# hsp-iit/online-detection

Measured on AMD Instinct MI355X. Metric: FALKON fit+infer samples/sec (N=1e6 D=1024 M=1e4), higher is better.
Workload: dtype f32-accurate K_nM (X Z' as a two-term f16 split on the f16 MFMA, f32 accumulate) stored as 24-bit fixed point (step 2^-24) + f64 solver (preconditioner: K_MM, T and T^-1 in f64; the products of the A factor, which only preconditions, at f32 accuracy on the f16 MFMA)

## Files before the change

online-detection_amd/csrc/knm_pass_q.hip:

```cpp
#include <algorithm>
#include <stdlib.h>

#include "odx_internal.h"
#include "knm_q.h"

namespace odx {

template <int NT, int CH, int R, int NV, int FMT, int WPE>
__device__ __forceinline__ void knm_passq_body(const unsigned short* __restrict__ Khi, int64_t ldk,
                                               const unsigned char* __restrict__ Klo, int64_t ldlo, int64_t n,
                                               int64_t M, const double* __restrict__ v1, const double* __restrict__ v2,
                                               const double* __restrict__ w, double* __restrict__ slab, int64_t slab_ld,
                                               double* __restrict__ t_out, int wg, int nwg, int64_t Mv = 0,
                                               const int* __restrict__ cstart = nullptr, const int* __restrict__ cpos = nullptr) {
  constexpr int NW = NT / 64;
  constexpr int CW = QCW;
  extern __shared__ __attribute__((aligned(16))) double vsq[];
  __shared__ double red[2][NW][NV * R];
  const int tid = threadIdx.x, lane = tid & 63, wave = tid >> 6;
  const int nchunk = (int)((M + CW - 1) / CW);
  const int vcap = (nchunk + 1) * CW;
  const int64_t nblk = (n + R - 1) / R;
  const double vscale = FMT == QF_U24 ? 5.9604644775390625e-08 : 1.0;
  for (int i = tid; i < vcap; i += NT) {
    vsq[i] = (v1 != nullptr && i < M) ? q_v_entry(v1, i, Mv, cstart, cpos) * vscale : 0.0;
    if (NV == 2) vsq[vcap + i] = i < M ? q_v_entry(v2, i, Mv, cstart, cpos) * vscale : 0.0;
  }
  double acc[NV][CH][CW];
#pragma unroll
  for (int q = 0; q < NV; ++q)
#pragma unroll
    for (int c = 0; c < CH; ++c)
#pragma unroll
      for (int e = 0; e < CW; ++e) acc[q][c][e] = 0.0;

  QChunk<FMT, CW> kr[R][CH];
  const int rowb_hi = (int)ldk * 2, rowb_lo = (int)ldlo;
  const int voff_hi = tid * (2 * CW), voff_lo = tid * CW;
  __amdgpu_buffer_rsrc_t rs_hi, rs_lo;
  int rows_open = R;
  auto open_block = [&](int64_t blk) {
    const int64_t row0 = blk * R;
    rows_open = (int)(n - row0 < R ? n - row0 : R);
    rs_hi = __builtin_amdgcn_make_buffer_rsrc(const_cast<unsigned short*>(Khi + row0 * ldk), (short)0, rows_open * rowb_hi, 0x00020000);
    if (FMT == QF_U24)
      rs_lo = __builtin_amdgcn_make_buffer_rsrc(const_cast<unsigned char*>(Klo + row0 * ldlo), (short)0, rows_open * rowb_lo, 0x00020000);
  };
  auto load_block = [&](int c) {
#pragma unroll
    for (int r = 0; r < R; ++r) {
      const int rr = r < rows_open ? r : rows_open - 1;
      const u32x2q th = __builtin_amdgcn_raw_buffer_load_b64(rs_hi, voff_hi, rr * rowb_hi + c * (NT * 2 * CW), 0);
      kr[r][c].hi[0] = th[0], kr[r][c].hi[1] = th[1];
      if (FMT == QF_U24) kr[r][c].lo[0] = __builtin_amdgcn_raw_buffer_load_b32(rs_lo, voff_lo, rr * rowb_lo + c * (NT * CW), 0);
    }
  };

  int64_t blk = wg;
  if (blk < nblk) {
    open_block(blk);
#pragma unroll
    for (int c = 0; c < CH; ++c) load_block(c);
  }
  __syncthreads();
  int pp = 0;
  for (; blk < nblk; blk += nwg) {
    double t[NV][R];
#pragma unroll
    for (int q = 0; q < NV; ++q)
#pragma unroll
      for (int r = 0; r < R; ++r) t[q][r] = 0.0;
    if (v1 != nullptr) {
      int zofs;
      asm volatile("v_mov_b32 %0, 0" : "=v"(zofs));
#pragma unroll
      for (int c = 0; c < CH; ++c) {
#pragma unroll
        for (int q = 0; q < NV; ++q) {
          const int ch = tid + c * NT + zofs;
          const int vi = (ch < nchunk ? ch : nchunk) * CW;
          double vv[CW];
#pragma unroll
          for (int u = 0; u < CW / 2; ++u) {
            const f64x2q a = *reinterpret_cast<const f64x2q*>(&vsq[q * vcap + vi + 2 * u]);
            vv[2 * u] = a[0];
            vv[2 * u + 1] = a[1];
          }
#pragma unroll
          for (int r = 0; r < R; ++r)
#pragma unroll
            for (int e = 0; e < CW; ++e) t[q][r] = fma(q_entry<FMT, CW>(kr[r][c], e), vv[e], t[q][r]);
        }
        __builtin_amdgcn_sched_barrier(0);
      }
#pragma unroll
      for (int q = 0; q < NV; ++q)
#pragma unroll
        for (int r = 0; r < R; ++r) {
          double s = t[q][r];
#pragma unroll
          for (int off = 32; off > 0; off >>= 1) s += __shfl_xor(s, off);
          if (lane == 0) red[pp][wave][q * R + r] = s;
        }
      __syncthreads();
#pragma unroll
      for (int q = 0; q < NV; ++q)
#pragma unroll
        for (int r = 0; r < R; ++r) {
          double s = 0.0;
#pragma unroll
          for (int u = 0; u < NW; ++u) s += red[pp][u][q * R + r];
          t[q][r] = s;
        }
      pp ^= 1;
    }
    if (t_out != nullptr) {
      if (tid == 0) {
#pragma unroll
        for (int r = 0; r < R; ++r)
          if (blk * R + r < n) t_out[blk * R + r] = t[0][r];
      }
    }
#pragma unroll
    for (int r = 0; r < R; ++r) {
      const int64_t row = blk * R + r;
      if (row >= n) {
#pragma unroll
        for (int q = 0; q < NV; ++q) t[q][r] = 0.0;
      } else if (NV == 1 && w != nullptr) {
        t[0][r] += w[row];
      }
    }
#pragma unroll
    for (int c = 0; c < CH; ++c)
#pragma unroll
      for (int r = 0; r < R; ++r) {
#pragma unroll
        for (int u = 0; u < CW / 2; ++u) asm volatile("" : "+v"(kr[r][c].hi[u]));
        if (FMT == QF_U24) {
#pragma unroll
          for (int u = 0; u < CW / 4; ++u) asm volatile("" : "+v"(kr[r][c].lo[u]));
        }
      }
    const int64_t nxt = blk + nwg;
    if (nxt < nblk) open_block(nxt);
#pragma unroll
    for (int c = 0; c < CH; ++c) {
#pragma unroll
      for (int r = 0; r < R; ++r)
#pragma unroll
        for (int e = 0; e < CW; ++e) {
          const double kd = q_entry<FMT, CW>(kr[r][c], e);
#pragma unroll
          for (int q = 0; q < NV; ++q) acc[q][c][e] = fma(kd, t[q][r], acc[q][c][e]);
        }
      load_block(c);
      __builtin_amdgcn_sched_barrier(0);
    }
  }
  double* my = slab + (int64_t)wg * slab_ld * NV;
#pragma unroll
  for (int q = 0; q < NV; ++q)
#pragma unroll
    for (int c = 0; c < CH; ++c) {
      const int ch = tid + c * NT;
      if (ch < nchunk) {
#pragma unroll
        for (int e = 0; e < CW; ++e)
          if ((int64_t)ch * CW + e < slab_ld) my[q * slab_ld + (int64_t)ch * CW + e] = acc[q][c][e] * vscale;
      }
    }
}

template <int NT, int CH, int R, int NV, int FMT, int WPE>
__global__ __launch_bounds__(NT, WPE) void knm_passq_kernel(const unsigned short* __restrict__ Khi, int64_t ldk,
                                                       const unsigned char* __restrict__ Klo, int64_t ldlo, int64_t n,
                                                       int64_t M, const double* __restrict__ v1, const double* __restrict__ v2,
                                                       const double* __restrict__ w, double* __restrict__ slab, int64_t slab_ld,
                                                       double* __restrict__ t_out, int64_t Mv, const int* __restrict__ cstart,
                                                       const int* __restrict__ cpos) {
  knm_passq_body<NT, CH, R, NV, FMT, WPE>(Khi, ldk, Klo, ldlo, n, M, v1, v2, w, slab, slab_ld, t_out, (int)blockIdx.x, (int)gridDim.x, Mv,
                                          cstart, cpos);
}

struct PassBatchQ {
  const unsigned short* Khi[ODX_MAX_ZBATCH];
  const unsigned char* Klo[ODX_MAX_ZBATCH];
  int64_t ldk[ODX_MAX_ZBATCH];
  int64_t ldlo[ODX_MAX_ZBATCH];
  int64_t n[ODX_MAX_ZBATCH];
  int M[ODX_MAX_ZBATCH];
  int grid[ODX_MAX_ZBATCH];
};

template <int NT, int CH, int R, int FMT, int WPE = (NT >= 1024 ? 4 : 2)>
__global__ __launch_bounds__(NT, WPE) void knm_passq_batched_kernel(PassBatchQ pb, const double* __restrict__ v, int64_t vstride,
                                                                    double* __restrict__ slab, int64_t slab_ld, int64_t slab_stride) {
  const int b = blockIdx.y;
  if ((int)blockIdx.x >= pb.grid[b]) return;
  knm_passq_body<NT, CH, R, 1, FMT, WPE>(pb.Khi[b], pb.ldk[b], pb.Klo[b], pb.ldlo[b], pb.n[b], pb.M[b], v + (int64_t)b * vstride, nullptr,
                                         nullptr, slab + (int64_t)b * slab_stride, slab_ld, nullptr, (int)blockIdx.x, pb.grid[b]);
}

template <int CH, int R, int FMT>
__device__ __forceinline__ void knm_passq_stag_body(const unsigned short* __restrict__ Khi, int64_t ldk,
                                                    const unsigned char* __restrict__ Klo, int64_t ldlo, int64_t n,
                                                    int64_t M, const double* __restrict__ v1,
                                                    const double* __restrict__ w, double* __restrict__ slab,
                                                    int64_t slab_ld, double* __restrict__ t_out, int wg, int nwg,
                                                    int64_t Mv = 0, const int* __restrict__ cstart = nullptr,
                                                    const int* __restrict__ cpos = nullptr) {
  constexpr int NT = 256, CW = QCW;
  extern __shared__ __attribute__((aligned(16))) double vsq[];
  __shared__ double red[2][2][4][R];
  const int tid = threadIdx.x, lane = tid & 63;
  const int h = __builtin_amdgcn_readfirstlane(tid >> 8), hw = __builtin_amdgcn_readfirstlane((tid >> 6) & 3);
  const int ht = tid & 255;
  const int nchunk = (int)((M + CW - 1) / CW);
  constexpr int vcap = CH * NT * CW;
  const int64_t nblk = (n + R - 1) / R;
  const double vscale = FMT == QF_U24 ? 5.9604644775390625e-08 : 1.0;
  for (int i = tid; i < vcap; i += 512) vsq[i] = (v1 != nullptr && i < M) ? q_v_entry(v1, i, Mv, cstart, cpos) * vscale : 0.0;
  const int voff_hi = ht * (2 * CW), voff_lo = ht * CW;
  double acc[CH][CW];
#pragma unroll
  for (int c = 0; c < CH; ++c)
#pragma unroll
    for (int e = 0; e < CW; ++e) acc[c][e] = 0.0;
  QChunk<FMT, CW> kr[R][CH];
  const int rowb_hi = (int)ldk * 2, rowb_lo = (int)ldlo;
  __amdgpu_buffer_rsrc_t rs_hi, rs_lo;
  int rows_open = R;
  auto open_block = [&](int64_t blk) {
    const int64_t row0 = blk * R;
    rows_open = (int)(n - row0 < R ? n - row0 : R);
    rs_hi = __builtin_amdgcn_make_buffer_rsrc(const_cast<unsigned short*>(Khi + row0 * ldk), (short)0, rows_open * rowb_hi, 0x00020000);
    if (FMT == QF_U24)
      rs_lo = __builtin_amdgcn_make_buffer_rsrc(const_cast<unsigned char*>(Klo + row0 * ldlo), (short)0, rows_open * rowb_lo, 0x00020000);
  };
  auto load_block = [&](int c) {
#pragma unroll
    for (int r = 0; r < R; ++r) {
      const int rr = r < rows_open ? r : rows_open - 1;
      const u32x2q th = __builtin_amdgcn_raw_buffer_load_b64(rs_hi, voff_hi, rr * rowb_hi + c * (NT * 2 * CW), 0);
      kr[r][c].hi[0] = th[0], kr[r][c].hi[1] = th[1];
      if (FMT == QF_U24) kr[r][c].lo[0] = __builtin_amdgcn_raw_buffer_load_b32(rs_lo, voff_lo, rr * rowb_lo + c * (NT * CW), 0);
    }
  };
  __shared__ unsigned int arrived[2];
  if (tid < 2) arrived[tid] = 0u;
  const int64_t first = 2 * (int64_t)wg + h, step = 2 * (int64_t)nwg;
  const int64_t mine = first < nblk ? (nblk - first + step - 1) / step : 0;
  if (mine > 0) {
    open_block(first);
#pragma unroll
    for (int c = 0; c < CH; ++c) load_block(c);
  }
  __syncthreads();
  int pp = 0;
  for (int64_t k = 0; k < mine; ++k) {
    const int64_t blk = first + k * step;
    double t[R];
#pragma unroll
    for (int r = 0; r < R; ++r) t[r] = 0.0;
    if (v1 != nullptr) {
      int zofs;
      asm volatile("v_mov_b32 %0, 0" : "=v"(zofs));
#pragma unroll
      for (int c = 0; c < CH; ++c) {
        const int vi = (ht + c * NT + zofs) * CW;
        const f64x2q a = *reinterpret_cast<const f64x2q*>(&vsq[vi]);
        const f64x2q b = *reinterpret_cast<const f64x2q*>(&vsq[vi + 2]);
        const double v0 = a[0], v1_ = a[1], v2_ = b[0], v3 = b[1];
#pragma unroll
        for (int r = 0; r < R; ++r) {
          t[r] = fma(q_entry<FMT, CW>(kr[r][c], 0), v0, t[r]);
          t[r] = fma(q_entry<FMT, CW>(kr[r][c], 1), v1_, t[r]);
          t[r] = fma(q_entry<FMT, CW>(kr[r][c], 2), v2_, t[r]);
          t[r] = fma(q_entry<FMT, CW>(kr[r][c], 3), v3, t[r]);
        }
        __builtin_amdgcn_sched_barrier(0);
      }
#pragma unroll
      for (int r = 0; r < R; ++r) {
        double sum = t[r];
#pragma unroll
        for (int off = 32; off > 0; off >>= 1) sum += __shfl_xor(sum, off);
        if (lane == 0) red[h][pp][hw][r] = sum;
      }
      asm volatile("" ::: "memory");
      if (lane == 0) {
        __hip_atomic_fetch_add(&arrived[h], 1u, __ATOMIC_RELAXED, __HIP_MEMORY_SCOPE_WORKGROUP);
        const unsigned int want = 4u * (unsigned int)(k + 1);
        bool met = false;
        for (int spin = 0; spin < (1 << 26); ++spin) {
          if (__hip_atomic_load(&arrived[h], __ATOMIC_RELAXED, __HIP_MEMORY_SCOPE_WORKGROUP) >= want) { met = true; break; }
          __builtin_amdgcn_s_sleep(1);
        }
        if (!met) __builtin_trap();
      }
      __builtin_amdgcn_wave_barrier();
      asm volatile("" ::: "memory");
#pragma unroll
      for (int r = 0; r < R; ++r) t[r] = ((red[h][pp][0][r] + red[h][pp][1][r]) + red[h][pp][2][r]) + red[h][pp][3][r];
      pp ^= 1;
#pragma unroll
      for (int c = 0; c < CH; ++c)
#pragma unroll
        for (int r = 0; r < R; ++r) {
          asm volatile("" : "+v"(kr[r][c].hi[0]));
          asm volatile("" : "+v"(kr[r][c].hi[1]));
          if (FMT == QF_U24) asm volatile("" : "+v"(kr[r][c].lo[0]));
        }
    }
    if (t_out != nullptr && hw == 0) {
      if (lane == 0) {
#pragma unroll
        for (int r = 0; r < R; ++r)
          if (blk * R + r < n) t_out[blk * R + r] = t[r];
      }
    }
#pragma unroll
    for (int r = 0; r < R; ++r) {
      const int64_t row = blk * R + r;
      if (row >= n) t[r] = 0.0;
      else if (w != nullptr) t[r] += w[row];
    }
    const bool more = k + 1 < mine;
    if (more) open_block(blk + step);
#pragma unroll
    for (int c = 0; c < CH; ++c) {
#pragma unroll
      for (int r = 0; r < R; ++r)
#pragma unroll
        for (int e = 0; e < CW; ++e) acc[c][e] = fma(q_entry<FMT, CW>(kr[r][c], e), t[r], acc[c][e]);
      load_block(c);
      __builtin_amdgcn_sched_barrier(0);
    }
  }
  double* my = slab + (2 * (int64_t)wg + h) * slab_ld;
#pragma unroll
  for (int c = 0; c < CH; ++c) {
    const int ch = ht + c * NT;
    if (ch < nchunk) {
#pragma unroll
      for (int e = 0; e < CW; ++e)
        if ((int64_t)ch * CW + e < slab_ld) my[(int64_t)ch * CW + e] = acc[c][e] * vscale;
    }
  }
}

template <int CH, int R, int FMT>
__global__ __launch_bounds__(512, 2) void knm_passq_stag_kernel(const unsigned short* __restrict__ Khi, int64_t ldk,
                                                                const unsigned char* __restrict__ Klo, int64_t ldlo, int64_t n,
                                                                int64_t M, const double* __restrict__ v1,
                                                                const double* __restrict__ w, double* __restrict__ slab,
                                                                int64_t slab_ld, double* __restrict__ t_out, int64_t Mv,
                                                                const int* __restrict__ cstart, const int* __restrict__ cpos) {
  knm_passq_stag_body<CH, R, FMT>(Khi, ldk, Klo, ldlo, n, M, v1, w, slab, slab_ld, t_out, (int)blockIdx.x, (int)gridDim.x, Mv, cstart, cpos);
}

template <int CH, int R, int FMT>
__global__ __launch_bounds__(512, 2) void knm_passq_stag_batched_kernel(PassBatchQ pb, const double* __restrict__ v, int64_t vstride,
                                                                        double* __restrict__ slab, int64_t slab_ld,
                                                                        int64_t slab_stride) {
  const int b = blockIdx.y;
  if ((int)blockIdx.x >= pb.grid[b]) return;
  knm_passq_stag_body<CH, R, FMT>(pb.Khi[b], pb.ldk[b], pb.Klo[b], pb.ldlo[b], pb.n[b], pb.M[b], v + (int64_t)b * vstride, nullptr,
                                  slab + (int64_t)b * slab_stride, slab_ld, nullptr, (int)blockIdx.x, pb.grid[b]);
}

struct QCfg {
  int nt, ch, r, wg_per_cu;
};

static bool pick_qcfg(int64_t M, int nv, int fmt, QCfg* cfg) {
  const int64_t chunks = (M + 3) / 4;
  if (nv == 1) {
    if (chunks <= 256) { *cfg = {256, 1, 16, 2}; return true; }
    if (chunks <= 512) { *cfg = {0, 2, 8, 2}; return true; }
    if (chunks <= 1024) { *cfg = {0, 4, 4, 2}; return true; }
    if (chunks <= 2048) { *cfg = {256, 8, 3, 2}; return true; }
    if (chunks <= 2560) { *cfg = {0, 10, 2, 1}; return true; }
    if (chunks <= 3072) { *cfg = {512, 6, 4, 1}; return true; }
    if (chunks <= 5110) { *cfg = {1024, 5, 1, 1}; return true; }
    return false;
  }
  if (chunks <= 1024 || chunks > 2560) return false;
  if (chunks <= 2048) *cfg = {512, 4, 2, 1};
  else *cfg = {512, 5, 2, 1};
  const int64_t lds = 2 * (chunks + 1) * 4 * 8 + 2 * (cfg->nt / 64) * cfg->r * 2 * 8 + 64;
  return lds <= 163840;
}

static int g_pass_cus = 0;

int pass_cus() { return g_pass_cus > 0 ? g_pass_cus : workspace_cus(); }

static int qgrid_for(const QCfg& cfg, int64_t n) {
  const int cus = pass_cus();
  const int64_t nblk = cfg.nt == 0 ? ceil_div(ceil_div(n, cfg.r), 2) : ceil_div(n, cfg.r);
  int64_t g = (int64_t)cus * cfg.wg_per_cu;
  if (g > nblk) g = nblk;
  if (g < 1) g = 1;
  return (int)g;
}

template <int NV, int FMT>
static int dispatch_passq(const QCfg& cfg, const QBlock& b, int grid, size_t lds, hipStream_t s, const double* v, const double* v2,
                          const double* w, double* slab, int64_t slab_ld, double* t_out, const QCols& cm) {
#define ODX_Q(NT_, CH_, R_)                                                                                                      \
  return q_launch(knm_passq_kernel<NT_, CH_, R_, NV, FMT, (NT_ >= 1024 ? 4 : 2)>, dim3(grid), NT_, lds, s, b.hi, b.ldk, b.lo, b.ldlo, \
                  b.n, b.M, v, v2, w, slab, slab_ld, t_out, cm.Mv, cm.start, cm.pos)
#define ODX_QH(CH_, R_)                                                                                                          \
  return q_launch(knm_passq_stag_kernel<CH_, R_, FMT>, dim3(grid), 512, lds, s, b.hi, b.ldk, b.lo, b.ldlo, b.n, b.M, v, w, slab,  \
                  slab_ld, t_out, cm.Mv, cm.start, cm.pos)
  if constexpr (NV == 1) {
    if (cfg.nt == 0) {
      if (cfg.ch == 2) ODX_QH(2, 8);
      if (cfg.ch == 4) ODX_QH(4, 4);
      ODX_QH(10, 2);
    }
    if (cfg.nt == 256 && cfg.ch == 1) ODX_Q(256, 1, 16);
    if (cfg.nt == 256 && cfg.ch == 8) ODX_Q(256, 8, 3);
    if (cfg.nt == 512 && cfg.ch == 6) ODX_Q(512, 6, 4);
    ODX_Q(1024, 5, 1);
  } else {
    if (cfg.ch == 4) ODX_Q(512, 4, 2);
    ODX_Q(512, 5, 2);
  }
#undef ODX_Q
#undef ODX_QH
}

int check_q_block(const char* who, const void* K, int64_t ldk, const void* Klo, int64_t ldlo, int fmt, int64_t M) {
  ODX_REQUIRE(fmt == ODX_KNM_U24 || fmt == ODX_KNM_BF16, "%s: storage format must be ODX_KNM_U24 or ODX_KNM_BF16 (got %d)", who, fmt);
  ODX_REQUIRE(K && ldk % 8 == 0 && ldk >= round_up(M, 8) && (reinterpret_cast<uintptr_t>(K) & 7u) == 0,
              "%s: K must be 8-byte aligned with ldk %% 8 == 0, ldk >= roundup(M, 8)", who);
  if (fmt == ODX_KNM_U24)
    ODX_REQUIRE(Klo && ldlo % 8 == 0 && ldlo >= round_up(M, 8) && (reinterpret_cast<uintptr_t>(Klo) & 3u) == 0,
                "%s: the low-byte plane must be 4-byte aligned with ldlo %% 8 == 0, ldlo >= roundup(M, 8)", who);
  return ODX_OK;
}

static bool passq_batch_cfg(int B, const int64_t* M, int fmt, QCfg* out) {
  QCfg c0 = {0, 0, 0, 0};
  for (int b = 0; b < B; ++b) {
    QCfg c;
    if (M[b] <= 0 || !pick_qcfg(M[b], 1, fmt, &c)) return false;
    if (b == 0) c0 = c;
    else if (c.nt != c0.nt || c.ch != c0.ch || c.r != c0.r) return false;
  }
  const bool built = (c0.nt == 0 && (c0.ch == 2 || c0.ch == 4 || c0.ch == 10)) ||
                     (c0.nt == 256 && (c0.ch == 1 || c0.ch == 8)) || (c0.nt == 512 && c0.ch == 6);
  if (out) *out = c0;
  return B > 0 && built;
}

static void passq_batch_geometry(int B, const int64_t* n, const int64_t* M, const QCfg& cfg, int* gmax, int64_t* slab_ld) {
  int g = 1;
  int64_t mm = 1;
  for (int b = 0; b < B; ++b) {
    if (n[b] > 0) g = std::max(g, qgrid_for(cfg, n[b]));
    mm = std::max(mm, M[b]);
  }
  *gmax = g;
  *slab_ld = round_up(mm, 4);
}

int64_t knm_passq_batched_workspace_bytes(int B, const int64_t* n, const int64_t* M, int fmt) {
  QCfg cfg;
  if (!q_format(fmt) || !passq_batch_cfg(B, M, fmt, &cfg)) return ODX_ERR_UNSUPPORTED;
  int gmax;
  int64_t slab_ld;
  passq_batch_geometry(B, n, M, cfg, &gmax, &slab_ld);
  return (int64_t)B * (cfg.nt == 0 ? 2 : 1) * gmax * slab_ld * (int64_t)sizeof(double);
}

template <int FMT>
static int launch_passq_batched(const QCfg& cfg, const PassBatchQ& pb, int gmax, int B, size_t lds, hipStream_t s, const double* v,
                                int64_t vstride, double* slab, int64_t slab_ld, int64_t slab_stride) {
#define ODX_QB(NT_, CH_, R_) \
  return q_launch(knm_passq_batched_kernel<NT_, CH_, R_, FMT>, dim3(gmax, B), NT_, lds, s, pb, v, vstride, slab, slab_ld, slab_stride)
#define ODX_QBH(CH_, R_) \
  return q_launch(knm_passq_stag_batched_kernel<CH_, R_, FMT>, dim3(gmax, B), 512, lds, s, pb, v, vstride, slab, slab_ld, slab_stride)
  if (cfg.nt == 0 && cfg.ch == 2) ODX_QBH(2, 8);
  if (cfg.nt == 0 && cfg.ch == 4) ODX_QBH(4, 4);
  if (cfg.nt == 0 && cfg.ch == 10) ODX_QBH(10, 2);
  if (cfg.nt == 256 && cfg.ch == 1) ODX_QB(256, 1, 16);
  if (cfg.nt == 256 && cfg.ch == 8) ODX_QB(256, 8, 3);
  if (cfg.nt == 512 && cfg.ch == 6) ODX_QB(512, 6, 4);
#undef ODX_QB
#undef ODX_QBH
  set_error("knm_passq_batched: no class-batched kernel for this pass configuration");
  return ODX_ERR_UNSUPPORTED;
}

int knm_passq_batched(int B, const void* const* Khi, const int64_t* ldk, const void* const* Klo, const int64_t* ldlo, int fmt,
                      const int64_t* n, const int64_t* M, const double* v, int64_t vstride, double* out, int64_t ostride,
                      void* workspace, int64_t workspace_bytes, hipStream_t s) {
  ODX_REQUIRE(B >= 1 && B <= ODX_MAX_ZBATCH, "knm_passq_batched: 1..%d classes", ODX_MAX_ZBATCH);
  QCfg cfg;
  ODX_REQUIRE(q_format(fmt) && passq_batch_cfg(B, M, fmt, &cfg),
              "knm_passq_batched: the classes of a batch must share one pass configuration");
  int gmax;
  int64_t slab_ld;
  passq_batch_geometry(B, n, M, cfg, &gmax, &slab_ld);
  const int per = cfg.nt == 0 ? 2 : 1;
  const int64_t slab_stride = (int64_t)per * gmax * slab_ld;
  ODX_PROPAGATE(require_workspace("knm_passq_batched", workspace, workspace_bytes, (int64_t)B * slab_stride * (int64_t)sizeof(double)));
  PassBatchQ pb;
  int nslab[ODX_MAX_ZBATCH];
  for (int b = 0; b < ODX_MAX_ZBATCH; ++b) {
    const bool on = b < B;
    pb.Khi[b] = on ? static_cast<const unsigned short*>(Khi[b]) : nullptr;
    pb.Klo[b] = (on && fmt == ODX_KNM_U24) ? static_cast<const unsigned char*>(Klo[b]) : nullptr;
    pb.ldk[b] = on ? ldk[b] : 0;
    pb.ldlo[b] = (on && fmt == ODX_KNM_U24) ? ldlo[b] : 0;
    pb.n[b] = on ? n[b] : 0;
    pb.M[b] = on ? (int)M[b] : 0;
    pb.grid[b] = (on && n[b] > 0) ? qgrid_for(cfg, n[b]) : 0;
    nslab[b] = per * pb.grid[b];
    if (on && n[b] > 0) ODX_PROPAGATE(check_q_block("knm_passq_batched", Khi[b], ldk[b], Klo ? Klo[b] : nullptr, ldlo ? ldlo[b] : 0, fmt, M[b]));
  }
  double* slab = static_cast<double*>(workspace);
  const size_t lds = (cfg.nt == 0 ? (size_t)(cfg.ch * 256 * 4) : (size_t)(slab_ld + 4)) * sizeof(double);
  if (fmt == ODX_KNM_U24) ODX_PROPAGATE((launch_passq_batched<QF_U24>(cfg, pb, gmax, B, lds, s, v, vstride, slab, slab_ld, slab_stride)));
  else ODX_PROPAGATE((launch_passq_batched<QF_BF16>(cfg, pb, gmax, B, lds, s, v, vstride, slab, slab_ld, slab_stride)));
  ODX_CHECK_LAUNCH("knm_passq_batched");
  return slab_reduce_batched_f64(B, M, nslab, slab, slab_ld, slab_stride, out, ostride, s);
}

}

using namespace odx;

extern "C" const char* odx_knm_pass_kernel_name(int64_t M, int fmt, int nv) {
  static thread_local char name[96];
  name[0] = 0;
  if (fmt == 0) {
    snprintf(name, sizeof(name), nv == 2 ? "knm_pass2_kernel" : "knm_pass_kernel");
    return name;
  }
  QCfg cfg;
  if ((fmt != QF_U24 && fmt != QF_BF16) || (nv != 1 && nv != 2) || M <= 0 || !pick_qcfg(M, nv, fmt, &cfg)) return name;
  if (cfg.nt == 0) snprintf(name, sizeof(name), "knm_passq_stag_kernel<%d,%d,%d>", cfg.ch, cfg.r, fmt);
  else snprintf(name, sizeof(name), "knm_passq_kernel<%d,%d,%d,%d,%d,%d>", cfg.nt, cfg.ch, cfg.r, nv, fmt, cfg.nt >= 1024 ? 4 : 2);
  return name;
}

extern "C" int odx_set_pass_cus(int cus) {
  ODX_REQUIRE(cus >= 0 && cus <= 4096, "odx_set_pass_cus: 0 (the device's) .. 4096");
  g_pass_cus = cus;
  return ODX_OK;
}

extern "C" int64_t odx_knm_fwd_bwd_q_workspace_bytes(int64_t n, int64_t M, int fmt) {
  QCfg cfg;
  if (n <= 0 || M <= 0) return 0;
  if (!q_format(fmt) || !pick_qcfg(M, 1, fmt, &cfg)) return ODX_ERR_UNSUPPORTED;
  return (int64_t)workspace_cus() * (cfg.nt == 0 ? 2 * cfg.wg_per_cu : cfg.wg_per_cu) * round_up(M, 4) * (int64_t)sizeof(double);
}

static int check_q_cols(const char* who, const QCols& cm, int64_t M) {
  ODX_REQUIRE(cm.Mv >= M && cm.Mv <= INT32_MAX && cm.col_of && cm.start && cm.pos, "%s: needs Mv >= M and col_of, start, pos", who);
  return ODX_OK;
}

static int knm_fwd_bwd_q_impl(const void* K, int64_t ldk, const void* Klo, int64_t ldlo, int fmt, int64_t n, int64_t M,
                              const double* v, const double* w, double* out, double* t_out, void* workspace,
                              int64_t workspace_bytes, odx_stream_t stream, const QCols& cm = QCols()) {
  ODX_REQUIRE(M > 0 && out, "odx_knm_fwd_bwd_q: M <= 0 or null out");
  hipStream_t s = as_stream(stream);
  if (n <= 0) {
    ODX_CHECK_HIP(hipMemsetAsync(out, 0, (size_t)(cm.on() ? cm.Mv : M) * sizeof(double), s));
    return ODX_OK;
  }
  ODX_REQUIRE(v || w, "odx_knm_fwd_bwd_q: both v and w null");
  ODX_PROPAGATE(check_q_block("odx_knm_fwd_bwd_q", K, ldk, Klo, ldlo, fmt, M));
  QCfg cfg;
  if (!pick_qcfg(M, 1, fmt, &cfg)) {
    set_error("odx_knm_fwd_bwd_q: M = %lld exceeds the %lld columns the compact-format pass kernels are built for", (long long)M,
              (long long)Q_MAX_M);
    return ODX_ERR_UNSUPPORTED;
  }
  const int grid = qgrid_for(cfg, n);
  const int64_t slab_ld = round_up(M, 4);
  const int nslab = cfg.nt == 0 ? 2 * grid : grid;
  ODX_PROPAGATE(require_workspace("odx_knm_fwd_bwd_q", workspace, workspace_bytes, (int64_t)nslab * slab_ld * (int64_t)sizeof(double)));
  double* slab = static_cast<double*>(workspace);
  const size_t lds = (cfg.nt == 0 ? (size_t)(cfg.ch * 256 * 4) : (size_t)(slab_ld + 4)) * sizeof(double);
  ODX_PROPAGATE(q_dispatch(q_block(K, ldk, Klo, ldlo, fmt, n, M), [&](auto f, const QBlock& b) {
    return dispatch_passq<1, decltype(f)::value>(cfg, b, grid, lds, s, v, nullptr, w, slab, slab_ld, t_out, cm);
  }));
  ODX_CHECK_LAUNCH("odx_knm_fwd_bwd_q");
  if (cm.on()) return slab_reduce_cols_f64(slab, slab_ld, nslab, 1, M, cm.Mv, cm.col_of, out, nullptr, s);
  return slab_reduce_f64(slab, slab_ld, nslab, M, out, s);
}

extern "C" int odx_knm_fwd_bwd_q(const void* K, int64_t ldk, const void* Klo, int64_t ldlo, int fmt, int64_t n, int64_t M,
                                 const double* v, const double* w, double* out, void* workspace, int64_t workspace_bytes,
                                 odx_stream_t stream) {
  return knm_fwd_bwd_q_impl(K, ldk, Klo, ldlo, fmt, n, M, v, w, out, nullptr, workspace, workspace_bytes, stream);
}

extern "C" int odx_knm_fwd_bwd_q_t(const void* K, int64_t ldk, const void* Klo, int64_t ldlo, int fmt, int64_t n, int64_t M,
                                   const double* v, const double* w, double* out, double* t_out, void* workspace,
                                   int64_t workspace_bytes, odx_stream_t stream) {
  ODX_REQUIRE(t_out == nullptr || v != nullptr, "odx_knm_fwd_bwd_q_t: t_out needs v");
  return knm_fwd_bwd_q_impl(K, ldk, Klo, ldlo, fmt, n, M, v, w, out, t_out, workspace, workspace_bytes, stream);
}

extern "C" int64_t odx_knm_fwd_bwd2_q_workspace_bytes(int64_t n, int64_t M, int fmt) {
  QCfg cfg;
  if (n <= 0 || M <= 0) return 0;
  if (!q_format(fmt) || !pick_qcfg(M, 2, fmt, &cfg)) return ODX_ERR_UNSUPPORTED;
  return 2 * (int64_t)workspace_cus() * cfg.wg_per_cu * round_up(M, 4) * (int64_t)sizeof(double);
}

static int knm_fwd_bwd2_q_impl(const void* K, int64_t ldk, const void* Klo, int64_t ldlo, int fmt, int64_t n, int64_t M,
                               const double* v, const double* v2, double* out, double* out2, double* t_out, void* workspace,
                               int64_t workspace_bytes, odx_stream_t stream, const QCols& cm = QCols()) {
  ODX_REQUIRE(M > 0 && out && out2, "odx_knm_fwd_bwd2_q: M <= 0 or null out");
  hipStream_t s = as_stream(stream);
  if (n <= 0) {
    ODX_CHECK_HIP(hipMemsetAsync(out, 0, (size_t)(cm.on() ? cm.Mv : M) * sizeof(double), s));
    ODX_CHECK_HIP(hipMemsetAsync(out2, 0, (size_t)(cm.on() ? cm.Mv : M) * sizeof(double), s));
    return ODX_OK;
  }
  ODX_REQUIRE(v && v2, "odx_knm_fwd_bwd2_q: null v or v2");
  ODX_PROPAGATE(check_q_block("odx_knm_fwd_bwd2_q", K, ldk, Klo, ldlo, fmt, M));
  QCfg cfg;
  if (!pick_qcfg(M, 2, fmt, &cfg)) {
    set_error("odx_knm_fwd_bwd2_q: M = %lld is outside the two-vector configurations (use two single passes)", (long long)M);
    return ODX_ERR_UNSUPPORTED;
  }
  const int grid = qgrid_for(cfg, n);
  const int64_t slab_ld = round_up(M, 4);
  ODX_PROPAGATE(require_workspace("odx_knm_fwd_bwd2_q", workspace, workspace_bytes, 2 * (int64_t)grid * slab_ld * (int64_t)sizeof(double)));
  double* slab = static_cast<double*>(workspace);
  const size_t lds = (size_t)(2 * (slab_ld + 4) * sizeof(double));
  ODX_PROPAGATE(q_dispatch(q_block(K, ldk, Klo, ldlo, fmt, n, M), [&](auto f, const QBlock& b) {
    return dispatch_passq<2, decltype(f)::value>(cfg, b, grid, lds, s, v, v2, nullptr, slab, slab_ld, t_out, cm);
  }));
  ODX_CHECK_LAUNCH("odx_knm_fwd_bwd2_q");
  if (cm.on()) return slab_reduce_cols_f64(slab, slab_ld, grid, 2, M, cm.Mv, cm.col_of, out, out2, s);
  return slab_reduce2_f64(slab, slab_ld, grid, M, out, out2, s);
}

extern "C" int odx_knm_fwd_bwd2_q(const void* K, int64_t ldk, const void* Klo, int64_t ldlo, int fmt, int64_t n, int64_t M,
                                  const double* v, const double* v2, double* out, double* out2, void* workspace,
                                  int64_t workspace_bytes, odx_stream_t stream) {
  return knm_fwd_bwd2_q_impl(K, ldk, Klo, ldlo, fmt, n, M, v, v2, out, out2, nullptr, workspace, workspace_bytes, stream);
}

extern "C" int odx_knm_fwd_bwd2_q_t(const void* K, int64_t ldk, const void* Klo, int64_t ldlo, int fmt, int64_t n, int64_t M,
                                    const double* v, const double* v2, double* out, double* out2, double* t_out, void* workspace,
                                    int64_t workspace_bytes, odx_stream_t stream) {
  return knm_fwd_bwd2_q_impl(K, ldk, Klo, ldlo, fmt, n, M, v, v2, out, out2, t_out, workspace, workspace_bytes, stream);
}

extern "C" int odx_knm_fwd_bwd_q_cols_t(const void* K, int64_t ldk, const void* Klo, int64_t ldlo, int fmt, int64_t n, int64_t M,
                                        const double* v, const double* w, double* out, double* t_out, void* workspace,
                                        int64_t workspace_bytes, int64_t Mv, const int32_t* col_of, const int32_t* start,
                                        const int32_t* pos, odx_stream_t stream) {
  ODX_REQUIRE(t_out == nullptr || v != nullptr, "odx_knm_fwd_bwd_q_cols_t: t_out needs v");
  const QCols cm = {Mv, col_of, start, pos};
  ODX_PROPAGATE(check_q_cols("odx_knm_fwd_bwd_q_cols_t", cm, M));
  return knm_fwd_bwd_q_impl(K, ldk, Klo, ldlo, fmt, n, M, v, w, out, t_out, workspace, workspace_bytes, stream, cm);
}

extern "C" int odx_knm_fwd_bwd2_q_cols_t(const void* K, int64_t ldk, const void* Klo, int64_t ldlo, int fmt, int64_t n, int64_t M,
                                         const double* v, const double* v2, double* out, double* out2, double* t_out,
                                         void* workspace, int64_t workspace_bytes, int64_t Mv, const int32_t* col_of,
                                         const int32_t* start, const int32_t* pos, odx_stream_t stream) {
  const QCols cm = {Mv, col_of, start, pos};
  ODX_PROPAGATE(check_q_cols("odx_knm_fwd_bwd2_q_cols_t", cm, M));
  return knm_fwd_bwd2_q_impl(K, ldk, Klo, ldlo, fmt, n, M, v, v2, out, out2, t_out, workspace, workspace_bytes, stream, cm);
}
```

online-detection_amd/csrc/knm_q.h:

```cpp
#pragma once
#include <type_traits>

#include "odx_internal.h"

namespace odx {

typedef unsigned int u32x4q __attribute__((ext_vector_type(4)));
typedef unsigned int u32x2q __attribute__((ext_vector_type(2)));
typedef double f64x2q __attribute__((ext_vector_type(2)));

enum { QF_U24 = 1, QF_BF16 = 2 };

constexpr int QCW = 4;
template <int FMT, int CW>
struct QChunk {
  unsigned hi[CW / 2];
  unsigned lo[CW / 4];
};

template <int FMT, int CW>
__device__ __forceinline__ double q_entry(const QChunk<FMT, CW>& k, int e) {
  const unsigned h = k.hi[e >> 1];
  if (FMT == QF_U24) {
    const unsigned sel = ((e & 1) ? 0x0c070600u : 0x0c050400u) | (unsigned)(e & 3);
    return (double)__builtin_amdgcn_perm(h, k.lo[e >> 2], sel);
  }
  return (double)__uint_as_float((e & 1) ? (h & 0xffff0000u) : (h << 16));
}

struct QCols {
  int64_t Mv = 0;
  const int* col_of = nullptr;
  const int* start = nullptr;
  const int* pos = nullptr;
  bool on() const { return start != nullptr; }
};

__device__ __forceinline__ double cols_fold_entry(const double* __restrict__ v, int64_t d, int64_t Mv, const int* __restrict__ start,
                                                  const int* __restrict__ pos) {
  const int last = (int)Mv - 1;
  int k = start[d], e = start[d + 1];
  k = k < 0 ? 0 : k;
  e = e > (int)Mv ? (int)Mv : e;
  double s = 0.0;
  for (; k < e; ++k) {
    int j = pos[k];
    j = j < 0 ? 0 : (j > last ? last : j);
    s += v[j];
  }
  return s;
}

__device__ __forceinline__ double q_v_entry(const double* __restrict__ v, int64_t i, int64_t Mv, const int* __restrict__ start,
                                            const int* __restrict__ pos) {
  return start == nullptr ? v[i] : cols_fold_entry(v, i, Mv, start, pos);
}

struct QBlock {
  const unsigned short* hi;
  int64_t ldk;
  const unsigned char* lo;
  int64_t ldlo;
  int fmt;
  int64_t n, M;
};

inline QBlock q_block(const void* K, int64_t ldk, const void* Klo, int64_t ldlo, int fmt, int64_t n, int64_t M) {
  return {static_cast<const unsigned short*>(K), ldk, static_cast<const unsigned char*>(Klo), ldlo, fmt, n, M};
}

inline bool q_format(int fmt) { return fmt == ODX_KNM_U24 || fmt == ODX_KNM_BF16; }

template <typename F>
int q_dispatch(QBlock b, F&& f) {
  if (b.fmt == ODX_KNM_U24) return f(std::integral_constant<int, QF_U24>(), b);
  b.lo = nullptr, b.ldlo = 0;
  return f(std::integral_constant<int, QF_BF16>(), b);
}

template <typename... P, typename... A>
int q_launch(void (*kernel)(P...), dim3 grid, int threads, size_t lds, hipStream_t s, A... args) {
  if (lds > 0)
    ODX_CHECK_HIP(hipFuncSetAttribute(reinterpret_cast<const void*>(kernel), hipFuncAttributeMaxDynamicSharedMemorySize, (int)lds));
  hipLaunchKernelGGL(kernel, grid, dim3(threads), lds, s, args...);
  return ODX_OK;
}

constexpr int64_t Q_MAX_M = 20440;
inline int q_nvt(int nv) { return nv <= 2 ? 2 : nv <= 4 ? 4 : 8; }
inline bool q_nv_supported(int64_t M, int fmt, int nv) { return q_format(fmt) && M > 0 && M <= Q_MAX_M && nv >= 1 && nv <= 8; }
#define ODX_REQUIRE_Q_NV(who, M, fmt, nv)                                                                                          \
  do {                                                                                                                             \
    if (!q_nv_supported(M, fmt, nv)) {                                                                                             \
      set_error("%s: needs ODX_KNM_U24 or ODX_KNM_BF16, 1 <= M <= %lld and 1 <= nv <= 8 (got fmt %d, M %lld, nv %d)", who,         \
                (long long)Q_MAX_M, fmt, (long long)(M), nv);                                                                      \
      return ODX_ERR_UNSUPPORTED;                                                                                                  \
    }                                                                                                                              \
  } while (0)

inline int workspace_cus() {
  const int cus = odx_device_cus();
  return cus > 0 ? cus : 256;
}

inline int require_workspace(const char* who, const void* workspace, int64_t workspace_bytes, int64_t need) {
  if (workspace != nullptr && workspace_bytes >= need) return ODX_OK;
  set_error("%s: workspace too small", who);
  return ODX_ERR_WORKSPACE;
}

inline int reduce_nv(int nv, int64_t M, int nslab, const double* slab, int64_t slab_ld, double* out, int64_t ldo, hipStream_t s) {
  int64_t Ms[8];
  int ns[8];
  for (int q = 0; q < nv; ++q) Ms[q] = M, ns[q] = nslab;
  return slab_reduce_batched_f64(nv, Ms, ns, slab, slab_ld, (int64_t)nslab * slab_ld, out, ldo, s);
}

}
```

Measured before the change: 193,600.

## Route two-vector K_nM pass with large M through staggered two-half kernel

For the NV=2, CH=5 configuration (M between 8192 and ~10240 columns), the pass kernel now dispatches to the staggered body, generalized to two vectors. The workgroup splits into two 256-thread halves that walk interleaved runs of 8 rows. Each half covers the full M range with 10 chunks per thread and skips chunks past the end. The two halves' accumulators are merged through LDS before the slab write, and t_out rows are batched per 8-row run. This aims to raise per-row parallelism and latency hiding in the dominant K_nM pass, at the cost of extra LDS, a final cross-half reduction, and more register pressure.

After: 193,900, median of 6. Within noise of the previous version (+0.1%).

```diff
diff --git a/online-detection_amd/csrc/knm_pass_q.hip b/online-detection_amd/csrc/knm_pass_q.hip
--- a/online-detection_amd/csrc/knm_pass_q.hip
+++ b/online-detection_amd/csrc/knm_pass_q.hip
@@ -172,17 +172,6 @@
     }
 }
 
-template <int NT, int CH, int R, int NV, int FMT, int WPE>
-__global__ __launch_bounds__(NT, WPE) void knm_passq_kernel(const unsigned short* __restrict__ Khi, int64_t ldk,
-                                                       const unsigned char* __restrict__ Klo, int64_t ldlo, int64_t n,
-                                                       int64_t M, const double* __restrict__ v1, const double* __restrict__ v2,
-                                                       const double* __restrict__ w, double* __restrict__ slab, int64_t slab_ld,
-                                                       double* __restrict__ t_out, int64_t Mv, const int* __restrict__ cstart,
-                                                       const int* __restrict__ cpos) {
-  knm_passq_body<NT, CH, R, NV, FMT, WPE>(Khi, ldk, Klo, ldlo, n, M, v1, v2, w, slab, slab_ld, t_out, (int)blockIdx.x, (int)gridDim.x, Mv,
-                                          cstart, cpos);
-}
-
 struct PassBatchQ {
   const unsigned short* Khi[ODX_MAX_ZBATCH];
   const unsigned char* Klo[ODX_MAX_ZBATCH];
@@ -202,31 +191,41 @@
                                          nullptr, slab + (int64_t)b * slab_stride, slab_ld, nullptr, (int)blockIdx.x, pb.grid[b]);
 }
 
-template <int CH, int R, int FMT>
+template <int CH, int R, int FMT, int NV = 1, int LOCH = 0>
 __device__ __forceinline__ void knm_passq_stag_body(const unsigned short* __restrict__ Khi, int64_t ldk,
                                                     const unsigned char* __restrict__ Klo, int64_t ldlo, int64_t n,
-                                                    int64_t M, const double* __restrict__ v1,
+                                                    int64_t M, const double* __restrict__ v1, const double* __restrict__ v2,
                                                     const double* __restrict__ w, double* __restrict__ slab,
                                                     int64_t slab_ld, double* __restrict__ t_out, int wg, int nwg,
                                                     int64_t Mv = 0, const int* __restrict__ cstart = nullptr,
                                                     const int* __restrict__ cpos = nullptr) {
   constexpr int NT = 256, CW = QCW;
+  constexpr int G = NV == 1 ? 1 : QRUN / R;
+  static_assert(NV == 1 || (G * R == QRUN && (G & (G - 1)) == 0), "a run is 8 rows: R must be 1, 2, 4 or 8");
+  constexpr int SURE = NV == 1 ? CH : LOCH / NT;
   extern __shared__ __attribute__((aligned(16))) double vsq[];
-  __shared__ double red[2][2][4][R];
+  __shared__ double red[2][2][4][NV * R];
+  __shared__ double trow[2][QRUN];
   const int tid = threadIdx.x, lane = tid & 63;
   const int h = __builtin_amdgcn_readfirstlane(tid >> 8), hw = __builtin_amdgcn_readfirstlane((tid >> 6) & 3);
   const int ht = tid & 255;
   const int nchunk = (int)((M + CW - 1) / CW);
-  constexpr int vcap = CH * NT * CW;
+  const int vcap = NV == 1 ? CH * NT * CW : (nchunk + 1) * CW;
   const int64_t nblk = (n + R - 1) / R;
   const double vscale = FMT == QF_U24 ? 5.9604644775390625e-08 : 1.0;
-  for (int i = tid; i < vcap; i += 512) vsq[i] = (v1 != nullptr && i < M) ? q_v_entry(v1, i, Mv, cstart, cpos) * vscale : 0.0;
+  for (int i = tid; i < vcap; i += 512) {
+    vsq[i] = (v1 != nullptr && i < M) ? q_v_entry(v1, i, Mv, cstart, cpos) * vscale : 0.0;
+    if (NV == 2) vsq[vcap + i] = i < M ? q_v_entry(v2, i, Mv, cstart, cpos) * vscale : 0.0;
+  }
   const int voff_hi = ht * (2 * CW), voff_lo = ht * CW;
-  double acc[CH][CW];
-#pragma unroll
-  for (int c = 0; c < CH; ++c)
-#pragma unroll
-    for (int e = 0; e < CW; ++e) acc[c][e] = 0.0;
+  double acc[NV][CH][CW];
+#pragma unroll
+  for (int q = 0; q < NV; ++q)
+#pragma unroll
+    for (int c = 0; c < CH; ++c)
+#pragma unroll
+      for (int e = 0; e < CW; ++e) acc[q][c][e] = 0.0;
+  auto walks = [&](int c) { return c < SURE || hw * 64 + c * NT < nchunk; };
   QChunk<FMT, CW> kr[R][CH];
   const int rowb_hi = (int)ldk * 2, rowb_lo = (int)ldlo;
   __amdgpu_buffer_rsrc_t rs_hi, rs_lo;
@@ -249,45 +248,74 @@
   };
   __shared__ unsigned int arrived[2];
   if (tid < 2) arrived[tid] = 0u;
+  const int64_t nrun = (nblk + G - 1) / G;
   const int64_t first = 2 * (int64_t)wg + h, step = 2 * (int64_t)nwg;
-  const int64_t mine = first < nblk ? (nblk - first + step - 1) / step : 0;
+  const int64_t runs = first < nrun ? (nrun - first + step - 1) / step : 0;
+  const int64_t mine = runs * G - ((runs > 0 && first + (runs - 1) * step == nrun - 1) ? nrun * G - nblk : 0);
+  auto block_of = [&](int64_t k) { return (first + (k / G) * step) * G + (k & (G - 1)); };
   if (mine > 0) {
-    open_block(first);
+    open_block(block_of(0));
 #pragma unroll
     for (int c = 0; c < CH; ++c) load_block(c);
   }
   __syncthreads();
   int pp = 0;
   for (int64_t k = 0; k < mine; ++k) {
-    const int64_t blk = first + k * step;
-    double t[R];
-#pragma unroll
-    for (int r = 0; r < R; ++r) t[r] = 0.0;
+    const int64_t blk = block_of(k);
+    double t[NV][R];
+#pragma unroll
+    for (int q = 0; q < NV; ++q)
+#pragma unroll
+      for (int r = 0; r < R; ++r) t[q][r] = 0.0;
     if (v1 != nullptr) {
       int zofs;
       asm volatile("v_mov_b32 %0, 0" : "=v"(zofs));
 #pragma unroll
       for (int c = 0; c < CH; ++c) {
-        const int vi = (ht + c * NT + zofs) * CW;
-        const f64x2q a = *reinterpret_cast<const f64x2q*>(&vsq[vi]);
-        const f64x2q b = *reinterpret_cast<const f64x2q*>(&vsq[vi + 2]);
-        const double v0 = a[0], v1_ = a[1], v2_ = b[0], v3 = b[1];
+        if constexpr (NV == 1) {
+          const int vi = (ht + c * NT + zofs) * CW;
+          const f64x2q a = *reinterpret_cast<const f64x2q*>(&vsq[vi]);
+          const f64x2q b = *reinterpret_cast<const f64x2q*>(&vsq[vi + 2]);
+          const double v0 = a[0], v1_ = a[1], v2_ = b[0], v3 = b[1];
+#pragma unroll
+          for (int r = 0; r < R; ++r) {
+            t[0][r] = fma(q_entry<FMT, CW>(kr[r][c], 0), v0, t[0][r]);
+            t[0][r] = fma(q_entry<FMT, CW>(kr[r][c], 1), v1_, t[0][r]);
+            t[0][r] = fma(q_entry<FMT, CW>(kr[r][c], 2), v2_, t[0][r]);
+            t[0][r] = fma(q_entry<FMT, CW>(kr[r][c], 3), v3, t[0][r]);
+          }
+        } else if (walks(c)) {
+          const int ch = ht + c * NT + zofs;
+          const int vi = (ch < nchunk ? ch : nchunk) * CW;
+          double vv[NV][CW];
+#pragma unroll
+          for (int q = 0; q < NV; ++q)
+#pragma unroll
+            for (int u = 0; u < CW / 2; ++u) {
+              const f64x2q a = *reinterpret_cast<const f64x2q*>(&vsq[q * vcap + vi + 2 * u]);
+              vv[q][2 * u] = a[0];
+              vv[q][2 * u + 1] = a[1];
+            }
+#pragma unroll
+          for (int r = 0; r < R; ++r)
+#pragma unroll
+            for (int e = 0; e < CW; ++e) {
+              const double kd = q_entry<FMT, CW>(kr[r][c], e);
+#pragma unroll
+              for (int q = 0; q < NV; ++q) t[q][r] = fma(kd, vv[q][e], t[q][r]);
+            }
+        }
+        __builtin_amdgcn_sched_barrier(0);
+      }
+#pragma unroll
+      for (int q = 0; q < NV; ++q)
 #pragma unroll
         for (int r = 0; r < R; ++r) {
-          t[r] = fma(q_entry<FMT, CW>(kr[r][c], 0), v0, t[r]);
-          t[r] = fma(q_entry<FMT, CW>(kr[r][c], 1), v1_, t[r]);
-          t[r] = fma(q_entry<FMT, CW>(kr[r][c], 2), v2_, t[r]);
-          t[r] = fma(q_entry<FMT, CW>(kr[r][c], 3), v3, t[r]);
-        }
-        __builtin_amdgcn_sched_barrier(0);
-      }
-#pragma unroll
-      for (int r = 0; r < R; ++r) {
-        double sum = t[r];
-#pragma unroll
-        for (int off = 32; off > 0; off >>= 1) sum += __shfl_xor(sum, off);
-        if (lane == 0) red[h][pp][hw][r] = sum;
-      }
+          double sum = t[q][r];
+#pragma unroll
+          for (int off = 32; off > 0; off >>= 1) sum += __shfl_xor(sum, off);
+          if (lane == 0) red[h][pp][hw][q * R + r] = sum;
+        }
       asm volatile("" ::: "memory");
       if (lane == 0) {
         __hip_atomic_fetch_add(&arrived[h], 1u, __ATOMIC_RELAXED, __HIP_MEMORY_SCOPE_WORKGROUP);
@@ -302,7 +330,12 @@
       __builtin_amdgcn_wave_barrier();
       asm volatile("" ::: "memory");
 #pragma unroll
-      for (int r = 0; r < R; ++r) t[r] = ((red[h][pp][0][r] + red[h][pp][1][r]) + red[h][pp][2][r]) + red[h][pp][3][r];
+      for (int q = 0; q < NV; ++q)
+#pragma unroll
+        for (int r = 0; r < R; ++r) {
+          const int i = q * R + r;
+          t[q][r] = ((red[h][pp][0][i] + red[h][pp][1][i]) + red[h][pp][2][i]) + red[h][pp][3][i];
+        }
       pp ^= 1;
 #pragma unroll
       for (int c = 0; c < CH; ++c)
@@ -313,40 +346,111 @@
           if (FMT == QF_U24) asm volatile("" : "+v"(kr[r][c].lo[0]));
         }
     }
-    if (t_out != nullptr && hw == 0) {
+    if constexpr (G == 1) {
+      if (t_out != nullptr && hw == 0) {
+        if (lane == 0) {
+#pragma unroll
+          for (int r = 0; r < R; ++r)
+            if (blk * R + r < n) t_out[blk * R + r] = t[0][r];
+        }
+      }
+    } else if (t_out != nullptr && hw == 0) {
+      const int g = (int)(k & (G - 1));
       if (lane == 0) {
 #pragma unroll
-        for (int r = 0; r < R; ++r)
-          if (blk * R + r < n) t_out[blk * R + r] = t[r];
+        for (int r = 0; r < R; ++r) trow[h][g * R + r] = t[0][r];
+      }
+      if (g == G - 1 || k + 1 == mine) {
+        asm volatile("" ::: "memory");
+        const int64_t row = (blk - g) * R + lane;
+        if (lane < QRUN && row < n) t_out[row] = trow[h][lane];
       }
     }
 #pragma unroll
     for (int r = 0; r < R; ++r) {
       const int64_t row = blk * R + r;
-      if (row >= n) t[r] = 0.0;
-      else if (w != nullptr) t[r] += w[row];
+      if (row >= n) {
+#pragma unroll
+        for (int q = 0; q < NV; ++q) t[q][r] = 0.0;
+      } else if (NV == 1 && w != nullptr) {
+        t[0][r] += w[row];
+      }
     }
     const bool more = k + 1 < mine;
-    if (more) open_block(blk + step);
+    if (more) open_block(block_of(k + 1));
 #pragma unroll
     for (int c = 0; c < CH; ++c) {
-#pragma unroll
-      for (int r = 0; r < R; ++r)
-#pragma unroll
-        for (int e = 0; e < CW; ++e) acc[c][e] = fma(q_entry<FMT, CW>(kr[r][c], e), t[r], acc[c][e]);
+      if (walks(c)) {
+#pragma unroll
+        for (int r = 0; r < R; ++r)
+#pragma unroll
+          for (int e = 0; e < CW; ++e) {
+            const double kd = q_entry<FMT, CW>(kr[r][c], e);
+#pragma unroll
+            for (int q = 0; q < NV; ++q) acc[q][c][e] = fma(kd, t[q][r], acc[q][c][e]);
+          }
+      }
       load_block(c);
       __builtin_amdgcn_sched_barrier(0);
     }
   }
-  double* my = slab + (2 * (int64_t)wg + h) * slab_ld;
-#pragma unroll
-  for (int c = 0; c < CH; ++c) {
-    const int ch = ht + c * NT;
-    if (ch < nchunk) {
-#pragma unroll
-      for (int e = 0; e < CW; ++e)
-        if ((int64_t)ch * CW + e < slab_ld) my[(int64_t)ch * CW + e] = acc[c][e] * vscale;
-    }
+  if constexpr (NV == 1) {
+    double* my = slab + (2 * (int64_t)wg + h) * slab_ld;
+#pragma unroll
+    for (int c = 0; c < CH; ++c) {
+      const int ch = ht + c * NT;
+      if (ch < nchunk) {
+#pragma unroll
+        for (int e = 0; e < CW; ++e)
+          if ((int64_t)ch * CW + e < slab_ld) my[(int64_t)ch * CW + e] = acc[0][c][e] * vscale;
+      }
+    }
+  } else {
+    __syncthreads();
+    if (h == 1) {
+#pragma unroll
+      for (int q = 0; q < NV; ++q)
+#pragma unroll
+        for (int c = 0; c < CH; ++c) {
+          const int ch = ht + c * NT;
+          if (ch < nchunk) {
+#pragma unroll
+            for (int e = 0; e < CW; ++e) vsq[q * vcap + ch * CW + e] = acc[q][c][e];
+          }
+        }
+    }
+    __syncthreads();
+    if (h == 0) {
+      double* my = slab + (int64_t)wg * slab_ld * NV;
+#pragma unroll
+      for (int q = 0; q < NV; ++q)
+#pragma unroll
+        for (int c = 0; c < CH; ++c) {
+          const int ch = ht + c * NT;
+          if (ch < nchunk) {
+#pragma unroll
+            for (int e = 0; e < CW; ++e)
+              if ((int64_t)ch * CW + e < slab_ld)
+                my[q * slab_ld + (int64_t)ch * CW + e] = (acc[q][c][e] + vsq[q * vcap + ch * CW + e]) * vscale;
+          }
+        }
+    }
+  }
+}
+
+template <int NT, int CH, int R, int NV, int FMT, int WPE>
+__global__ __launch_bounds__(NT, WPE) void knm_passq_kernel(const unsigned short* __restrict__ Khi, int64_t ldk,
+                                                       const unsigned char* __restrict__ Klo, int64_t ldlo, int64_t n,
+                                                       int64_t M, const double* __restrict__ v1, const double* __restrict__ v2,
+                                                       const double* __restrict__ w, double* __restrict__ slab, int64_t slab_ld,
+                                                       double* __restrict__ t_out, int64_t Mv, const int* __restrict__ cstart,
+                                                       const int* __restrict__ cpos) {
+  if constexpr (NV == 2 && NT == 512 && CH == 5 && R == 2) {
+    knm_passq_stag_body<10, 1, FMT, 2, 2048>(Khi, ldk, Klo, ldlo, n, M, v1, v2, nullptr, slab, slab_ld, t_out, (int)blockIdx.x,
+                                             (int)gridDim.x, Mv, cstart, cpos);
+  } else {
+    knm_passq_body<NT, CH, R, NV, FMT, WPE>(Khi, ldk, Klo, ldlo, n, M, v1, v2, w, slab, slab_ld, t_out, (int)blockIdx.x, (int)gridDim.x, Mv,
+                                            cstart, cpos);
   }
 }
 
@@ -357,7 +461,7 @@
                                                                 const double* __restrict__ w, double* __restrict__ slab,
                                                                 int64_t slab_ld, double* __restrict__ t_out, int64_t Mv,
                                                                 const int* __restrict__ cstart, const int* __restrict__ cpos) {
-  knm_passq_stag_body<CH, R, FMT>(Khi, ldk, Klo, ldlo, n, M, v1, w, slab, slab_ld, t_out, (int)blockIdx.x, (int)gridDim.x, Mv, cstart, cpos);
+  knm_passq_stag_body<CH, R, FMT>(Khi, ldk, Klo, ldlo, n, M, v1, nullptr, w, slab, slab_ld, t_out, (int)blockIdx.x, (int)gridDim.x, Mv, cstart, cpos);
 }
 
 template <int CH, int R, int FMT>
@@ -367,11 +471,12 @@
   const int b = blockIdx.y;
   if ((int)blockIdx.x >= pb.grid[b]) return;
   knm_passq_stag_body<CH, R, FMT>(pb.Khi[b], pb.ldk[b], pb.Klo[b], pb.ldlo[b], pb.n[b], pb.M[b], v + (int64_t)b * vstride, nullptr,
-                                  slab + (int64_t)b * slab_stride, slab_ld, nullptr, (int)blockIdx.x, pb.grid[b]);
+                                  nullptr, slab + (int64_t)b * slab_stride, slab_ld, nullptr, (int)blockIdx.x, pb.grid[b]);
 }
 
 struct QCfg {
   int nt, ch, r, wg_per_cu;
+  bool halves2 = false;
 };
 
 static bool pick_qcfg(int64_t M, int nv, int fmt, QCfg* cfg) {
@@ -388,8 +493,9 @@
   }
   if (chunks <= 1024 || chunks > 2560) return false;
   if (chunks <= 2048) *cfg = {512, 4, 2, 1};
-  else *cfg = {512, 5, 2, 1};
-  const int64_t lds = 2 * (chunks + 1) * 4 * 8 + 2 * (cfg->nt / 64) * cfg->r * 2 * 8 + 64;
+  else *cfg = {512, 5, 2, 1, true};
+  const int64_t fixed = cfg->halves2 ? (2 * 2 * 4 * 2 + 2 * QRUN) * 8 + 8 : 2 * (cfg->nt / 64) * cfg->r * 2 * 8;
+  const int64_t lds = 2 * (chunks + 1) * 4 * 8 + fixed + 64;
   return lds <= 163840;
 }
 
@@ -399,7 +505,7 @@
 
 static int qgrid_for(const QCfg& cfg, int64_t n) {
   const int cus = pass_cus();
-  const int64_t nblk = cfg.nt == 0 ? ceil_div(ceil_div(n, cfg.r), 2) : ceil_div(n, cfg.r);
+  const int64_t nblk = cfg.halves2 ? ceil_div(ceil_div(n, QRUN), 2) : cfg.nt == 0 ? ceil_div(ceil_div(n, cfg.r), 2) : ceil_div(n, cfg.r);
   int64_t g = (int64_t)cus * cfg.wg_per_cu;
   if (g > nblk) g = nblk;
   if (g < 1) g = 1;
diff --git a/online-detection_amd/csrc/knm_q.h b/online-detection_amd/csrc/knm_q.h
--- a/online-detection_amd/csrc/knm_q.h
+++ b/online-detection_amd/csrc/knm_q.h
@@ -12,6 +12,7 @@
 enum { QF_U24 = 1, QF_BF16 = 2 };
 
 constexpr int QCW = 4;
+constexpr int QRUN = 8;
 template <int FMT, int CW>
 struct QChunk {
   unsigned hi[CW / 2];
```
